# ultravideo/kvazaar

Measured on AMD Instinct MI355X. Metric: CTUs/s (all-intra ultrafast hot path), higher is better.
Workload: dtype u8/i16 (f64 RD costs); 1 GPU; 1920x1080 yuv420p 8-bit all-intra ultrafast CTU pass (kvz_hip_intra_frames), QP 22; ctus_per_frame=510, distinct_frames=8, wpp=True, parallelism=frames sharded over 1 GPU(s), no data-path collective

## Files before the change

include/kvz_hip_dev.h:

```cpp
#ifndef KVZ_HIP_DEV_H_
#define KVZ_HIP_DEV_H_

#include "kvz_hip_types.h"

#ifdef __cplusplus
extern "C" {
#endif

void *kvz_hip_dev_alloc(size_t bytes);
void  kvz_hip_dev_free(void *p);
void  kvz_hip_dev_upload(void *dev_dst, const void *host_src, size_t bytes);
void  kvz_hip_dev_download(void *host_dst, const void *dev_src, size_t bytes);
void  kvz_hip_dev_sync(void);
void  kvz_hip_dev_copy(void *dev_dst, const void *dev_src, size_t bytes);
void  kvz_hip_dev_timer_start(void);
float kvz_hip_dev_timer_stop(void);

int  kvz_hip_dev_sad_nxn(int n, const uint8_t *a, const uint8_t *b, int count, uint32_t *out);
int  kvz_hip_dev_satd_nxn(int n, const uint8_t *a, const uint8_t *b, int count, uint32_t *out);

int  kvz_hip_dev_transform(int kind, const int16_t *in, int16_t *tmp, int16_t *out, int count, int use_matrix_cores);

int  kvz_hip_dev_angular_pred(int log2_width, int mode, const uint8_t *ref_above, const uint8_t *ref_left, int count, uint8_t *out);

int  kvz_hip_dev_intra_select(int log2w, int nblk, const uint32_t *raw, const int8_t *preds, const double *mode_bits, int count, int32_t *winner);

int  kvz_hip_dev_cu8_units(int count, int from_coeffs, const int16_t *in, const int32_t *qp, int16_t *levels, int16_t *dequant, int16_t *resid);

int  kvz_hip_dev_satd8_blocks(const uint8_t *a, const uint8_t *b, int count, uint32_t *out);

int  kvz_hip_dev_rough_rows(int log2w, const uint8_t *top, const uint8_t *left, int count, uint8_t *out);

void kvz_hip_dev_deblock_frames(uint8_t *frames, int width, int height, int n_frames, const uint8_t *cu_depth, int qp, int beta_offset_div2,
                                int tc_offset_div2);

typedef struct kvz_hip_cu_dbk {
  uint8_t type;
  uint8_t depth, tr_depth, part_size;
  uint8_t cbf_y;
  uint8_t mv_dir;
  int8_t  mv_ref[2];
  int16_t ref_id[2];
  int16_t mv[2][2];
} kvz_hip_cu_dbk;
void kvz_hip_dev_deblock_frames_inter(uint8_t *frames, int width, int height, int n_frames, const kvz_hip_cu_dbk *info, int qp, int beta_offset_div2,
                                      int tc_offset_div2, int slice_is_b);

int  kvz_hip_dev_loop_filters_inter(const uint8_t *src, uint8_t *rec, int width, int height, int n_pictures, const kvz_hip_cu_dbk *info, int qp, int slice_is_b, int deblock,
                                    int beta_offset_div2, int tc_offset_div2, int sao, int no_wpp, kvz_hip_sao_params *luma, kvz_hip_sao_params *chroma, uint8_t *merge);

int  kvz_hip_dev_sad_surface(const uint8_t *cur, const uint8_t *ref, int width, int height, int bw, int range, const int16_t *blk_xy, int count,
                             uint32_t *out);

typedef struct kvz_hip_fme_pu {
// ... 123 lines not shown
```

kvazaar_amd/csrc/kvz_ctu.hpp:

```cpp
#pragma once
#include <type_traits>
#include "../../include/kvz_hip_types.h"
#include "kvz_ops.hpp"
#include "kvz_rdoq.hpp"
#include "kvz_recon.hpp"
#include "kvz_residual.hpp"
#include "kvz_select.hpp"

namespace kvz {

#define KVZ_CTU_THREADS 128
#ifdef KVZ_HOSTSIM
#define KVZ_FOR_THREADS(tid) for (int tid = 0; tid < KVZ_CTU_THREADS; ++tid)
#ifdef KVZ_HOSTSIM_COUNT_SYNCS
static unsigned long long g_kvz_syncs;
#define KVZ_SYNC() (++g_kvz_syncs)
#else
#define KVZ_SYNC()
#endif
#define KVZ_LDS_ADD(p, v) (*(p) += (v))
#else
#define KVZ_FOR_THREADS(tid) for (int tid = (threadIdx.x + lane_rot) & (KVZ_CTU_THREADS - 1), once_ = 1; once_; once_ = 0)
#define KVZ_SYNC() __syncthreads()
#define KVZ_LDS_ADD(p, v) atomicAdd((p), (v))
// ... 233 lines not shown
  u8 dcval[3];
  int8_t mode_disp[35];
  int16_t mode_inv[35];
  QuantScalars qs[4][2];
  double mode_bits_cost[3];
  CtxSetT<CABAC> cab, pre[3], post2;
  float entropy_fbits[128];
  u8 ctx_lps[64];
};

using CtuShared = CtuSharedT<true>;
static_assert(__builtin_offsetof(CtuSharedT<true>, fref) == __builtin_offsetof(CtuSharedT<true>, ref) + 408 && __builtin_offsetof(CtuSharedT<false>, fref) == __builtin_offsetof(CtuSharedT<false>, ref) + 408,
              "Tables::mref_tab addresses the filtered references 408 bytes behind the unfiltered ones");
static_assert(KVZ_MREF_STRIDE == kMrefStride && KVZ_MREF_ORG == kMrefOrg && sizeof(((CtuSharedT<true> *)0)->ref[0][0]) == kMrefRefRow && kMrefFiltered == 408,
              "Tables::mref_tab (kvz_tables.hpp) is built for this layout of the reference arrays");
#define KVZ_FROM_REF(T, member) (__builtin_offsetof(T, member) - __builtin_offsetof(T, ref))
static_assert(KVZ_FROM_REF(CtuSharedT<true>, mref) == kMrefExtended && KVZ_FROM_REF(CtuSharedT<false>, mref) == kMrefExtended && KVZ_FROM_REF(CtuSharedT<true>, org_t) == kSatdSrcT &&
              KVZ_FROM_REF(CtuSharedT<false>, org_t) == kSatdSrcT && KVZ_FROM_REF(CtuSharedT<true>, edge_x) == kSatdEdge && KVZ_FROM_REF(CtuSharedT<false>, edge_x) == kSatdEdge,
              "Tables::satd_rows (kvz_tables.hpp) addresses the extended references, the transposed source block and the edge bytes from CtuShared::ref");
static_assert(sizeof(((CtuSharedT<true> *)0)->edge_x) >= 1 + 2 * 16 && __builtin_offsetof(CtuSharedT<true>, edge_x) + sizeof(((CtuSharedT<true> *)0)->edge_x) <= __builtin_offsetof(CtuSharedT<true>, lv2_coeff) &&
              __builtin_offsetof(CtuSharedT<true>, org) == 0 && __builtin_offsetof(CtuSharedT<true>, ref) % 8 == 0 && __builtin_offsetof(CtuSharedT<true>, org_t) % 8 == 0,
              "the edge bytes of a 16x16 CU fit, behind satd_raw and inside the union; source rows (offsets that are multiples of 8 from org / org_t) are 8-byte aligned");
static_assert(__builtin_offsetof(CtuSharedT<true>, lv2_coeff) - __builtin_offsetof(CtuSharedT<true>, tb_big) == 3072 + 1536, "the union is as large as its 32x32 regime: edge_x added nothing");
#undef KVZ_FROM_REF
static_assert(KVZ_CTU_THREADS == 128, "two wavefronts per CTU: thread 64 is 'the other wavefront' (recon_cu8, eval_pu, wide_task, rdoq_unit, prices_coeffs, kHookThread), a 16x16 CU's "
                                      "128 (mode, block) pairs are one round of rough_search, plane_sums routes DPP rows per wavefront, and mref_pre[4] covers Tables::mref_tab's 510 entries");

KVZ_HD int plane_off(int c) { return c ? 3072 + (c << 10) : 0; }

struct RdoqLds {
  i32 ptab[2 * 148];
  u8 diag8[64];
  u8 mode4[4][64][4];
  u8 nb_mode4_left[16];
  u8 c4[96];
  alignas(8) i16 lv4_coeff[96];
  u8 pu_mode[4], pu_cbf[4];
  int pu_cbf_c[2];
  int a3x, a3y, n_pu;
  double split_cost3;
  CtxSetT<true> pre3, post3;
};
template <bool CABAC, bool S32 = false, bool RDOQ = false, bool SH = false, bool LISTS = false> struct CtuProgramT {
  static_assert(!(SH && RDOQ), "kvz_rdoq's own sign hiding is not built");
  static_assert(!(LISTS && (RDOQ || SH)), "scaling lists with kvz_rdoq or sign data hiding are not built");
  using CtxSet = CtxSetT<CABAC>;
// ... 1321 lines not shown
    if (lv == 3) return levels_lds(lv, c);
    return lv == 2 ? s->lv2_coeff + (c == 0 ? 0 : (c == 1 ? 256 : 320))
         : lv == 1 ? s->lv1_coeff + (c == 0 ? 0 : (c == 1 ? 1024 : 1280)) : coeff_level(lv) + plane_off(c) + ctu_zorder(xl >> sh, yl >> sh);
  }

  KVZ_DEV static int wide_trips(int lw) { return lw == 4 ? 1 : 2; }
  KVZ_DEV static RowPlan wide_rows(int lw, int trip) { return lw == 4 ? ROWS_W16 : (trip == 0 ? ROWS_W32_Y : ROWS_W32_C); }
  KVZ_DEV static int wide_task(int lw, int trip, int tid, int *seg)
  {
    *seg = 0;
    if (lw == 4) {
      if (tid < 32) { *seg = tid; return 0; }
      if (tid >= 64 || (tid & 15) >= 8) return -1;
      *seg = tid & 7;
      return tid < 48 ? 1 : 2;
    }
    if (trip == 0) { *seg = tid; return 0; }
    if (tid >= 64) return -1;
    *seg = tid & 31;
    return 1 + (tid >> 5);
  }
  KVZ_DEV void predict_row8(int l2, int mode, int c, int px0, int py, u8 out[8]) const
  {
    const int w = 1 << l2;
    const bool edges = c == 0 && w < 32;
    const u8 *top = s->ref[c][0], *left = s->ref[c][1];
    if (c == 0 && luma_reads_filtered(l2, mode)) { top = s->fref[0]; left = s->fref[1]; }
    if (mode == 0) {
      const int l = left[py + 1], tr = top[w + 1], bl = left[w + 1];
      const int hb = (w - 1) * l + tr + (py + 1) * bl + w, dl = tr - l, wy = w - 1 - py;
      for (int k = 0; k < 8; k++) out[k] = (u8)(((px0 + k) * dl + top[px0 + k + 1] * wy + hb) >> (l2 + 1));
    } else if (mode == 1) {
      const int dc = s->dcval[c];
      for (int k = 0; k < 8; k++) out[k] = (u8)dc;
      if (edges) {
        if (py == 0) for (int k = 0; k < 8; k++) out[k] = (u8)((top[px0 + k + 1] + 3 * dc + 2) >> 2);
        if (px0 == 0) out[0] = (u8)(py == 0 ? (left[1] + 2 * dc + top[1] + 2) >> 2 : (left[py + 1] + 3 * dc + 2) >> 2);
      }
    } else {
      const int disp = s->mode_disp[mode], inv = s->mode_inv[mode];
      const bool vertical = mode >= 18;
      const u8 *main_ref = vertical ? top : left, *side_ref = vertical ? left : top;
      if (vertical) {
        const int delta = (py + 1) * disp, di = delta >> 5, df = delta & 31;
        int r[9];
        if (disp >= 0) for (int j = 0; j < 9; j++) r[j] = main_ref[px0 + di + j + 1];
        else for (int j = 0; j < 9; j++) r[j] = angular_ref(main_ref, side_ref, px0 + di + j, inv);
        for (int k = 0; k < 8; k++) out[k] = (u8)(((32 - df) * r[k] + df * r[k + 1] + 16) >> 5);
        if (edges && mode == 26 && px0 == 0) out[0] = (u8)iclip(0, 255, (int)out[0] + ((left[py + 1] - left[0]) >> 1));
      } else {
        for (int k = 0; k < 8; k++) {
          const int delta = (px0 + k + 1) * disp, di = delta >> 5, df = delta & 31;
          const int r1 = disp >= 0 ? (int)main_ref[py + di + 1] : angular_ref(main_ref, side_ref, py + di, inv);
          const int r2 = disp >= 0 ? (int)main_ref[py + di + 2] : angular_ref(main_ref, side_ref, py + di + 1, inv);
          int v = ((32 - df) * r1 + df * r2 + 16) >> 5;
          if (edges && mode == 10 && py == 0) v = iclip(0, 255, v + ((top[px0 + k + 1] - top[0]) >> 1));
          out[k] = (u8)v;
        }
      }
    }
  }

  KVZ_DEV void predict_chroma_pair(int l2, int mode, int x, int y, u8 *pu, u8 *pv) const
  {
    const u8 *top_u = s->ref[1][0], *left_u = s->ref[1][1], *top_v = s->ref[2][0], *left_v = s->ref[2][1];
    if (mode == 0) { *pu = planar_pixel(l2, x, y, top_u, left_u); *pv = planar_pixel(l2, x, y, top_v, left_v); return; }
    if (mode == 1) { *pu = s->dcval[1]; *pv = s->dcval[2]; return; }
    const bool vertical = mode >= 18;
    const int px = vertical ? x : y, py = vertical ? y : x;
    const int delta_pos = (py + 1) * s->mode_disp[mode], di = delta_pos >> 5, df = delta_pos & 31, inv = s->mode_inv[mode];
    const int i1 = px + di, i2 = i1 + 1;
    const bool main1 = i1 >= -1, main2 = i2 >= -1;
    const int o1 = main1 ? i1 + 1 : (128 + (-1 - i1) * inv) >> 8, o2 = main2 ? i2 + 1 : (128 + (-1 - i2) * inv) >> 8;
    auto plane = [&](const u8 *top, const u8 *left) {
      const u8 *main_ref = vertical ? top : left, *side_ref = vertical ? left : top;
      const int r1 = (main1 ? main_ref : side_ref)[o1], r2 = (main2 ? main_ref : side_ref)[o2];
      return (u8)(((32 - df) * r1 + df * r2 + 16) >> 5);
    };
    *pu = plane(top_u, left_u);
    *pv = plane(top_v, left_v);
  }

  KVZ_DEV void recon_cu16(int lv, const TuSet &t, int depth, int mode)
  {
    const int xl = t.x - cx, yl = t.y - cy, xc = xl >> 1, yc = yl >> 1;
    const CandView cv = cand_view(lv);
    const int umode = uni(mode);
    const bool to_stage = cabac_on() && lv == 0;
    KVZ_LANE_VAR(WideBytes<16>, mat_f);
    KVZ_LANE_VAR(WideBytes<16>, mat_i);
    KVZ_LANE_VAR(u32, pred_org);
    KVZ_LANE_VAR(u32, coded);
#ifdef KVZ_HOSTSIM
#define KVZ_CU16_CODED(tid, c) ((void)KVZ_LANE(coded, tid), s->acc[6 + (c)] != 0)
#else
#define KVZ_CU16_CODED(tid, c) (((KVZ_LANE(coded, tid) >> ((c) == 2 ? 1 : 0)) & 1u) != 0)
#endif
    KVZ_FOR_THREADS(tid) {
      if (tid < 3) s->acc[3 * tid] = 0;
      if (tid >= 64 && tid < 70) s->acc[1 + (tid - 64) + ((tid - 64) >> 1)] = 0;
      if (tid < 32) {
        const int seg = mover_lane(tid), py = seg >> 1, px0 = (seg << 3) & 15;
        u8 p[8], o[8];
        i16 res[8];
        predict_row8(4, umode, 0, px0, py, p);
        __builtin_memcpy(o, KVZ_ALIGNED(org_at(0, xl + px0, yl + py), 8), 8);
        for (int k = 0; k < 8; k++) res[k] = (i16)((int)o[k] - (int)p[k]);
        __builtin_memcpy(KVZ_ALIGNED(&cv.at(0, xl + px0, yl + py), 8), p, 8);
        __builtin_memcpy(KVZ_ALIGNED(tbuf(t, 0, 0) + (seg << 3), 16), res, 16);
      } else if (tid >= 64) {
        const int e = tid - 64, px = e & 7, py = e >> 3;
        cu8_matrix_rows<3>(tb, e, KVZ_LANE(mat_f, tid), KVZ_LANE(mat_i, tid));
        u8 pu, pv;
        predict_chroma_pair(3, umode, px, py, &pu, &pv);
        cv.at(1, xc + px, yc + py) = pu;
        cv.at(2, xc + px, yc + py) = pv;
        const u8 ou = *org_at(1, xc + px, yc + py), ov = *org_at(2, xc + px, yc + py);
        KVZ_LANE(pred_org, tid) = (u32)pu | ((u32)ou << 8) | ((u32)pv << 16) | ((u32)ov << 24);
        tbuf(t, 0, 1)[e] = (i16)((int)ou - (int)pu);
        tbuf(t, 0, 2)[e] = (i16)((int)ov - (int)pv);
      }
    }
    KVZ_WAVE_SYNC();
    KVZ_PROF(KVZ_P_RPRED);
    KVZ_FOR_THREADS(tid) {
      if (tid < 64) transform_big(4, tbuf(t, 0, 0), false, tid, 0);
      else {
        const int e = tid - 64;
        tbuf(t, 1, 1)[e] = cu8_fwd_first<3>(tbuf(t, 0, 1), e, KVZ_LANE(mat_f, tid));
        tbuf(t, 1, 2)[e] = cu8_fwd_first<3>(tbuf(t, 0, 2), e, KVZ_LANE(mat_f, tid));
      }
    }
    KVZ_WAVE_SYNC();
    KVZ_PROF(KVZ_P_FDCT);
    KVZ_FOR_THREADS(tid) {
      const u32 cw_lo = (u32)uni((int)(u32)m->coeff_weights), cw_hi = (u32)uni((int)(u32)(m->coeff_weights >> 32));
      if (tid < 64) {
        u32 packed = 0;
        if (tid < 32) {
          const int seg = mover_lane(tid);
          const QuantScalars q = s->qs[2][0];
          i16 cf[8], lvl[8], dq[8];
          __builtin_memcpy(cf, KVZ_ALIGNED(tbuf(t, 0, 0) + (seg << 3), 16), 16);
          u32 wsum = 0, nz = 0;
          for (int k = 0; k < 8; k++) {
            ListFactor f{ 0, 0 };
            if constexpr (LISTS) f = factor_at(0, 4, (seg << 3) + k);
            const int level = LISTS ? quant_level(cf[k], q, f.fwd) : quant_level(cf[k], q);
            lvl[k] = (i16)level;
            const LevelCost lc = level_cost(level, cw_lo, cw_hi);
            wsum += lc.weight;
            nz += lc.nonzero;
            dq[k] = LISTS ? dequant_level(level, q, f.inv) : dequant_level(level, q);
          }
          packed = wsum | (nz << 24);
          __builtin_memcpy(KVZ_ALIGNED(coeff_dst(lv, 0, xl, yl) + (seg << 3), 16), lvl, 16);
          if (to_stage) __builtin_memcpy(KVZ_ALIGNED(levels_lds(lv, 0) + (seg << 3), 16), lvl, 16);
          __builtin_memcpy(KVZ_ALIGNED(tbuf(t, 1, 0) + (seg << 3), 16), dq, 16);
        }
        KVZ_LANE(coded, tid) = plane_sums(ROWS_CU16, tid, tid < 32 ? 0 : -1, packed, true, 3) != 0;
      } else {
        const int e = tid - 64;
        const QuantScalars q = s->qs[1][1];
        auto plane = [&](int c) {
          const int cf = cu8_fwd_second<3>(tbuf(t, 1, c), e, KVZ_LANE(mat_f, tid));
          ListFactor f{ 0, 0 };
          if constexpr (LISTS) f = factor_at(c, 3, e);
          const int level = LISTS ? quant_level(cf, q, f.fwd) : quant_level(cf, q);
          coeff_dst(lv, c, xl, yl)[e] = (i16)level;
          if (to_stage) levels_lds(lv, c)[e] = (i16)level;
          tbuf(t, 0, c)[cu8_transposed<3>(e)] = LISTS ? dequant_level(level, q, f.inv) : dequant_level(level, q);
          return level_cost(level, cw_lo, cw_hi).word();
        };
        const u32 wu = plane(1), wv = plane(2);
        const u32 nu = plane_sums(ROWS_CU16, tid, 1, wu, true, 3), nv = plane_sums(ROWS_CU16, tid, 2, wv, true, 3);
        KVZ_LANE(coded, tid) = (u32)(nu != 0) | ((u32)(nv != 0) << 1);
      }
    }
    KVZ_WAVE_SYNC();
    KVZ_PROF(KVZ_P_QUANT);
    KVZ_FOR_THREADS(tid) {
      if (tid < 64) { if (uni((int)KVZ_CU16_CODED(tid, 0))) transform_big(4, tbuf(t, 1, 0), true, tid, 0); }
      else {
        const int e = tid - 64;
        if (KVZ_CU16_CODED(tid, 1)) tbuf(t, 1, 1)[cu8_transposed<3>(e)] = cu8_inv_first<3>(tbuf(t, 0, 1), e, KVZ_LANE(mat_i, tid));
        if (KVZ_CU16_CODED(tid, 2)) tbuf(t, 1, 2)[cu8_transposed<3>(e)] = cu8_inv_first<3>(tbuf(t, 0, 2), e, KVZ_LANE(mat_i, tid));
      }
    }
    KVZ_WAVE_SYNC();
    KVZ_PROF(KVZ_P_IDCT);
    KVZ_FOR_THREADS(tid) {
      if (tid < 64) {
        u32 ssd = 0;
        if (tid < 32) {
          const int seg = mover_lane(tid), py = seg >> 1, px0 = (seg << 3) & 15;
          u8 *rp = &cv.at(0, xl + px0, yl + py);
          u8 v[8], o[8];
          __builtin_memcpy(v, KVZ_ALIGNED(rp, 8), 8);
          __builtin_memcpy(o, KVZ_ALIGNED(org_at(0, xl + px0, yl + py), 8), 8);
          if (KVZ_CU16_CODED(tid, 0)) {
            i16 res[8];
            __builtin_memcpy(res, KVZ_ALIGNED(tbuf(t, 1, 0) + (seg << 3), 16), 16);
            for (int k = 0; k < 8; k++) v[k] = (u8)recon_sample(v[k], res[k]);
            __builtin_memcpy(KVZ_ALIGNED(rp, 8), v, 8);
          }
          for (int k = 0; k < 8; k++) ssd += sq_err(o[k], v[k]);
        }
        plane_sums(ROWS_CU16, tid, tid < 32 ? 0 : -1, ssd, false, 0);
      } else {
        const int e = tid - 64, px = e & 7, py = e >> 3;
        auto plane = [&](int c) {
          const u32 po = KVZ_LANE(pred_org, tid) >> (c == 2 ? 16 : 0);
          int v = (int)(po & 0xffu);
          if (KVZ_CU16_CODED(tid, c)) {
            v = recon_sample(v, cu8_inv_second<3>(tbuf(t, 1, c), e, KVZ_LANE(mat_i, tid)));
            cv.at(c, xc + px, yc + py) = (u8)v;
          }
          return sq_err((int)((po >> 8) & 0xffu), v);
        };
        const u32 su = plane(1), sv = plane(2);
        plane_sums(ROWS_CU16, tid, 1, su, false, 0);
        plane_sums(ROWS_CU16, tid, 2, sv, false, 0);
      }
    }
#undef KVZ_CU16_CODED
    KVZ_SYNC();
    KVZ_FOR_THREADS(tid) {
      if (tid == 0) finish_planes(lv, xl, yl, depth, 0, 3, false);
    }
    if (cabac_on()) KVZ_SYNC();
    KVZ_PROF(KVZ_P_RECON);
// ... 23 lines not shown
          i16 res[8];
          predict_row8(l2, umode, c, px0, py, p);
          __builtin_memcpy(o, KVZ_ALIGNED(org_at(c, (xl >> sh) + px0, (yl >> sh) + py), 8), 8);
          for (int k = 0; k < 8; k++) res[k] = (i16)((int)o[k] - (int)p[k]);
          __builtin_memcpy(KVZ_ALIGNED(&cv.at(c, (xl >> sh) + px0, (yl >> sh) + py), 8), p, 8);
          __builtin_memcpy(KVZ_ALIGNED(tbuf(t, 0, c) + (seg << 3), 16), res, 16);
        }
      }
    } else
    KVZ_FOR_THREADS(tid) {
      if (tid < 16) s->acc[tid] = 0;
      for (int c = 0; c < 3; c++) {
        const int l2 = tu_log2(t, c), w = 1 << l2, sh = c ? 1 : 0;
        for (int e = tid; e < w * w; e += KVZ_CTU_THREADS) {
          const int px = e & (w - 1), py = e >> l2;
          const u8 p = predict_pixel(l2, mode, c, px, py);
          cv.at(c, (xl >> sh) + px, (yl >> sh) + py) = p;
          tbuf(t, 0, c)[e] = (i16)((int)*org_at(c, (xl >> sh) + px, (yl >> sh) + py) - (int)p);
        }
      }
    }
    KVZ_SYNC();
    KVZ_PROF(KVZ_P_RPRED);
    for (int pass = 0; pass < 2; pass++) {
      KVZ_FOR_THREADS(tid) {
        for (int c = 0; c < 3; c++) {
          const int l2 = tu_log2(t, c), n = 1 << l2;
          const i16 *src = tbuf(t, pass, c);
          i16 *dst = tbuf(t, pass ^ 1, c);
          if (l2 >= 4) {
            if (pass == 0 && !(big_pairs(t) && c == 2)) transform_big(l2, tbuf(t, 0, c), false, tid, c, big_pairs(t) && c == 1);
            continue;
          }
          for (int e = tid; e < n * n; e += KVZ_CTU_THREADS) {
            const int k = e >> l2, j = e & (n - 1);
            dst[e] = fwd_point(n, [&](int i) { return dct_at(l2, k, i); }, src, j << l2, pass == 0 ? l2 - 1 : l2 + 6);
          }
        }
      }
      KVZ_SYNC();
    }
    KVZ_PROF(KVZ_P_FDCT);
    if (RDOQ && m->rdoq) {
      KVZ_FOR_THREADS(tid) { rdoq_unit(tid, lv, t, true, depth, mode); }
      KVZ_SYNC();
      KVZ_PROF(KVZ_P_RDOQ);
    }
    if (SH && !RDOQ && wide && hide_on()) {
      auto held = [&](int c) { return lv == 0 ? levels_lds(lv, c) : coeff_dst(lv, c, xl, yl); };
      KVZ_FOR_THREADS(tid) {
        for (int trip = 0; trip < wide_trips(t.lw); trip++) {
          int seg;
          const int c = wide_task(t.lw, trip, mover_lane(tid), &seg);
          if (c < 0) continue;
          const QuantScalars q = s->qs[tu_log2(t, c) - 2][c ? 1 : 0];
          i16 cf[8], lvl[8];
          __builtin_memcpy(cf, KVZ_ALIGNED(tbuf(t, 0, c) + (seg << 3), 16), 16);
          for (int k = 0; k < 8; k++) lvl[k] = (i16)quant_level(cf[k], q);
          __builtin_memcpy(KVZ_ALIGNED(held(c) + (seg << 3), 16), lvl, 16);
        }
      }
      KVZ_SYNC();
      KVZ_FOR_THREADS(tid) { hide_signs(tid, t.lw, tu_log2(t, 1), intra_scan_order(mode, depth), tbuf(t, 0, 0), held(0), tbuf(t, 0, 1), held(1), tbuf(t, 0, 2), held(2)); }
// ... 79 lines not shown
        block_add(&s->acc[3 + c], wsum);
        block_add(&s->acc[6 + c], nz);
      }
    }
    KVZ_SYNC();
    KVZ_PROF(KVZ_P_QUANT);
    for (int pass = 0; pass < 2; pass++) {
      KVZ_FOR_THREADS(tid) {
        for (int c = 0; c < 3; c++) {
          const int l2 = tu_log2(t, c), n = 1 << l2;
          if (!s->acc[6 + c]) continue;
          const i16 *src = tbuf(t, pass ^ 1, c);
          i16 *dst = tbuf(t, pass, c);
          if (l2 >= 4) {
            if (pass == 0 && !(big_pairs(t) && c == 2 && s->acc[7])) transform_big(l2, tbuf(t, 1, c), true, tid, c, big_pairs(t) && c == 1 && s->acc[8]);
            continue;
          }
          for (int e = tid; e < n * n; e += KVZ_CTU_THREADS) {
            const int j = e >> l2, i = e & (n - 1);
            dst[e] = inv_point(n, [&](int k) { return dct_at(l2, k, i); }, src, j, n, pass == 0 ? 7 : 12);
          }
        }
      }
      KVZ_SYNC();
    }
    KVZ_PROF(KVZ_P_IDCT);
    KVZ_FOR_THREADS(tid) {
      if (wide) {
        for (int trip = 0; trip < wide_trips(t.lw); trip++) {
          int seg;
          const int c = wide_task(t.lw, trip, mover_lane(tid), &seg);
          u32 ssd = 0;
          if (c >= 0) {
            const int l2 = tu_log2(t, c), sh = c ? 1 : 0, py = seg >> (l2 - 3), px0 = (seg << 3) & ((1 << l2) - 1);
            u8 *rp = &cv.at(c, (xl >> sh) + px0, (yl >> sh) + py);
            u8 v[8], o[8];
            __builtin_memcpy(v, KVZ_ALIGNED(rp, 8), 8);
            __builtin_memcpy(o, KVZ_ALIGNED(org_at(c, (xl >> sh) + px0, (yl >> sh) + py), 8), 8);
            if (s->acc[6 + c] != 0) {
              i16 res[8];
              __builtin_memcpy(res, KVZ_ALIGNED(tbuf(t, 1, c) + (seg << 3), 16), 16);
              for (int k = 0; k < 8; k++) v[k] = (u8)recon_sample(v[k], res[k]);
              __builtin_memcpy(KVZ_ALIGNED(rp, 8), v, 8);
            }
            for (int k = 0; k < 8; k++) ssd += sq_err(o[k], v[k]);
          }
          plane_sums(wide_rows(t.lw, trip), tid, c, ssd, false, 0);
// ... 1106 lines not shown
```

kvazaar_amd/csrc/kvz_dev.hpp:

```cpp
#pragma once
#include <hip/hip_runtime.h>

#include <functional>
#include <mutex>
#include <chrono>
#include <vector>

#include "../../include/kvz_hip_dev.h"
#include "kvz_mfma.hpp"
#include "kvz_ops.hpp"
#include "kvz_sao.hpp"
#include "kvz_entropy.hpp"
#include "kvz_select.hpp"
#include "kvz_recon.hpp"
#include "kvz_tables.hpp"

namespace kvz {

__device__ __forceinline__ u32 load_u32_any(const u8 *p) { u32 v; __builtin_memcpy(&v, p, 4); return v; }
template <int G> __device__ __forceinline__ u32 group_sum(u32 v)
{
  for (int off = G / 2; off > 0; off >>= 1) v += __shfl_down(v, off, G);
  return v;
}
// ... 309 lines not shown
      const u8 xv = satd_edge_byte(ref0, L2, tid & (2 * W - 1));
      ref0[kSatdEdge + (tid == 2 * W ? 0 : 1 + tid)] = tid == 2 * W ? (u8)0 : xv;
    }
  }
  __syncthreads();
  if (!live || (L2 == 3 && tid >= 64)) return;
#pragma unroll
  for (int j = 0; j < (L2 == 4 ? 2 : 1); j++) {
    const int g = L2 == 4 ? 2 * (tid >> 6) + j : 0, pr = 32 * g + (lane & 31), mode = 2 + (pr >> LB), b = pr & (NBLK - 1);
    const dev_int4 *row = reinterpret_cast<const dev_int4 *>(tb->satd_rows[L2 == 4 ? 1 + g : 0][lane]);
    const dev_int4 e[2] = { row[0], row[1] };
    dev_int4 p[2];
    satd_rows_predict(ref0, e, p);
    u8 *o = out + ((cu * 32 + (mode - 2)) * NBLK + b) * 64;
#pragma unroll
    for (int i = 0; i < 4; i++)
#pragma unroll
      for (int x = 0; x < 8; x++) {
        const int r = 4 * (lane >> 5) + i;
        const u8 v = (u8)(((u32)p[i >> 1][2 * (i & 1) + (x >> 2)] >> (8 * (x & 3))) ^ 0x80);
        o[mode >= 18 ? 8 * r + x : 8 * x + r] = v;
      }
  }
}

template <int L2> __global__ void __launch_bounds__(256) dev_angular_kernel(const u8 *above, const u8 *left, const int count, const int mode, u8 *out)
{
  constexpr int W = 1 << L2, NG = kAngularGroupsPerLane, GPB = W * W / 4, BLOCKS = 256 * NG / GPB, RS = 2 * W + 1, ES = (2 * W + 1 + 8 + 3) & ~3;
  constexpr int RAW = (BLOCKS * RS + 3 + 3) / 4 + 2;
  __shared__ u32 s_raw[2][RAW];
  __shared__ alignas(8) u8 s_ext[BLOCKS][ES];
  __shared__ u32 s_tile[BLOCKS * W * W / 4];
  const int disp_tab[9] = { 0, 2, 5, 9, 13, 17, 21, 26, 32 };
  const int inv_tab[9] = { 0, 4096, 1638, 910, 630, 482, 390, 315, 256 };
  const bool vertical = mode >= 18;
  const int mode_disp = vertical ? mode - 26 : 10 - mode, ad = iabs(mode_disp);
  const int disp = mode_disp < 0 ? -disp_tab[ad] : disp_tab[ad], inv = inv_tab[ad];
  const long blk0 = (long)blockIdx.x * BLOCKS;
  const int nblk = (int)(count - blk0 < BLOCKS ? count - blk0 : BLOCKS);
  const long g0 = blk0 * RS;
  const int mis = (int)(g0 & 3), ndw = (mis + nblk * RS + 3) >> 2;
  const u8 *main_g = vertical ? above : left, *side_g = vertical ? left : above;
  const int tid = threadIdx.x;
  for (int i = tid; i < ndw; i += 256) {
    s_raw[0][i] = reinterpret_cast<const u32 *>(main_g + g0 - mis)[i];
    if (disp < 0) s_raw[1][i] = reinterpret_cast<const u32 *>(side_g + g0 - mis)[i];
// ... 857 lines not shown
}

int kvz_hip_dev_intra_select(int log2w, int nblk, const uint32_t *raw, const int8_t *preds, const double *mode_bits, int count, int32_t *winner)
{
  if (!((log2w == 3 && nblk == 1) || (log2w == 4 && nblk == 4))) { fprintf(stderr, "kvz_hip_dev_intra_select: unsupported log2w=%d nblk=%d\n", log2w, nblk); return -1; }
  if (count <= 0) return 0;
  KVZ_DEV_LAUNCH(kvz::dev_intra_select_kernel, ((long)count + 3) / 4 * 256, raw, preds, mode_bits, count, log2w, nblk, winner);
  return 0;
}

int kvz_hip_dev_cu8_units(int count, int from_coeffs, const int16_t *in, const int32_t *qp, int16_t *levels, int16_t *dequant, int16_t *resid)
{
  if (count < 0 || (from_coeffs != 0 && from_coeffs != 1)) { fprintf(stderr, "kvz_hip_dev_cu8_units: count=%d from_coeffs=%d\n", count, from_coeffs); return -1; }
  if (count == 0) return 0;
  KVZ_DEV_LAUNCH(kvz::dev_cu8_units_kernel, ((long)count + 1) / 2 * 256, in, qp, count, from_coeffs, kvz::device_tables(), levels, dequant, resid);
  return 0;
}

int kvz_hip_dev_rough_rows(int log2w, const uint8_t *top, const uint8_t *left, int count, uint8_t *out)
{
  if (count < 0 || (log2w != 3 && log2w != 4)) { fprintf(stderr, "kvz_hip_dev_rough_rows: log2w=%d count=%d\n", log2w, count); return -1; }
  if (log2w == 3) KVZ_DEV_LAUNCH(kvz::dev_rough_rows_kernel<3>, ((long)count + 1) / 2 * 256, kvz::device_tables(), top, left, count, out);
  else KVZ_DEV_LAUNCH(kvz::dev_rough_rows_kernel<4>, ((long)count + 1) / 2 * 256, kvz::device_tables(), top, left, count, out);
  return 0;
}

int kvz_hip_dev_satd8_blocks(const uint8_t *a, const uint8_t *b, int count, uint32_t *out)
{
  if (count < 0) { fprintf(stderr, "kvz_hip_dev_satd8_blocks: count=%d\n", count); return -1; }
  KVZ_DEV_LAUNCH(kvz::dev_satd8_blocks_kernel, ((long)count + 31) / 32 * 64, kvz::device_tables(), a, b, count, out);
  return 0;
}

void kvz_hip_dev_deblock_frames(uint8_t *frames, int width, int height, int n_frames, const uint8_t *cu_depth, int qp, int beta_offset_div2,
                                int tc_offset_div2)
{
  kvz::deblock_frames_on(be().stream, frames, width, height, n_frames, cu_depth, qp, beta_offset_div2, tc_offset_div2);
}

void kvz_hip_dev_deblock_frames_inter(uint8_t *frames, int width, int height, int n_frames, const kvz_hip_cu_dbk *info, int qp, int beta_offset_div2, int tc_offset_div2,
                                      int slice_is_b)
{
  kvz::deblock_frames_on(be().stream, frames, width, height, n_frames, nullptr, qp, beta_offset_div2, tc_offset_div2, 3, info, slice_is_b);
}

namespace kvz {
// ... 1027 lines not shown
```

kvazaar_amd/csrc/kvz_ops.hpp:

```cpp
#pragma once
#include <stdint.h>

#ifdef KVZ_HOSTSIM
#define KVZ_DEV inline
#define KVZ_ATOMIC_ADD(p, v) (*(p) += (v))
#else
#include <hip/hip_runtime.h>
#define KVZ_DEV __device__ __forceinline__
#define KVZ_ATOMIC_ADD(p, v) atomicAdd((p), (v))
#endif

namespace kvz {

typedef uint8_t u8;
typedef int16_t i16;
typedef uint16_t u16;
typedef uint32_t u32;
typedef int32_t i32;

#ifdef KVZ_HOSTSIM
#define KVZ_HD inline
#else
#define KVZ_HD __host__ __device__ __forceinline__
#endif
// ... 459 lines not shown
        const int scanpos = cg * cg_size + in_cg;
        const u32 blkpos = scan[scanpos];
        const int qv = quant_coeff[blkpos];
        int ld = imin(iabs((int)coef[blkpos]) * qv, 0x7fffffff - (1 << (q_bits - 1)));
        const u32 mx = (u32)((ld + (1 << (q_bits - 1))) >> q_bits);
        if (mx > 0) {
          res[0] = scanpos; res[1] = cg; res[2] = cg; res[3] = (scanpos > 0 && type == 0) ? 2 : 0; res[4] = (i32)blkpos;
          return;
        }
        dest[blkpos] = 0;
      }
    }
    res[2] = cg;
  }
};


KVZ_DEV int angular_ref(const u8 *main_ref, const u8 *side_ref, int i, int inv)
{
  const u8 *p = i >= -1 ? main_ref + (i + 1) : side_ref + ((128 + (-1 - i) * inv) >> 8);
  return *p;
}

KVZ_DEV u8 angular_pixel(int mode, int x, int y, const u8 *above, const u8 *left)
{
  const int disp_tab[9] = { 0, 2, 5, 9, 13, 17, 21, 26, 32 };
  const int inv_tab[9] = { 0, 4096, 1638, 910, 630, 482, 390, 315, 256 };
  const bool vertical = mode >= 18;
  const int mode_disp = vertical ? mode - 26 : 10 - mode;
  const int ad = iabs(mode_disp);
  const int sample_disp = mode_disp < 0 ? -disp_tab[ad] : disp_tab[ad];
  const u8 *main_ref = vertical ? above : left, *side_ref = vertical ? left : above;
  const int px = vertical ? x : y, py = vertical ? y : x;
  if (sample_disp == 0) return main_ref[px + 1];
  const int delta_pos = (py + 1) * sample_disp;
  const int di = delta_pos >> 5, df = delta_pos & 31;
  const int inv = inv_tab[ad];
  const int r1 = angular_ref(main_ref, side_ref, px + di, inv);
  if (!df) return (u8)r1;
  const int r2 = angular_ref(main_ref, side_ref, px + di + 1, inv);
  return (u8)(((32 - df) * r1 + df * r2 + 16) >> 5);
}

KVZ_DEV u8 planar_pixel(int log2w, int x, int y, const u8 *top, const u8 *left)
{
  const int w = 1 << log2w;
  const int hor = (w - 1 - x) * left[y + 1] + (x + 1) * top[w + 1];
  const int ver = (w - 1 - y) * top[x + 1] + (y + 1) * left[w + 1];
  return (u8)((ver + hor + w) >> (log2w + 1));
}

KVZ_DEV int dc_value(int log2w, const u8 *top, const u8 *left)
{
  const int w = 1 << log2w;
  int sum = 0;
  for (int i = 0; i < w; i++) sum += top[i + 1] + left[i + 1];
  return (u8)((sum + w) >> (log2w + 1));
}

KVZ_DEV u8 filtered_dc_pixel(int dc, int x, int y, const u8 *top, const u8 *left)
{
  if (x == 0 && y == 0) return (u8)((left[1] + 2 * dc + top[1] + 2) / 4);
  if (y == 0) return (u8)((top[x + 1] + 3 * dc + 2) / 4);
  if (x == 0) return (u8)((left[y + 1] + 3 * dc + 2) / 4);
  return (u8)dc;
}

struct IntraPredOp {
  int kind, log2w; const int8_t *modes ; const u8 *above; const u8 *left; long ref_bstride; u8 *dst;
  KVZ_DEV void operator()(int item) const
  {
    const int w = 1 << log2w, blk = item >> (2 * log2w), e = item & (w * w - 1), y = e >> log2w, x = e & (w - 1);
    const u8 *t = above + blk * ref_bstride, *l = left + blk * ref_bstride;
    u8 v;
    if (kind == 0) v = angular_pixel(modes[blk], x, y, t, l);
    else if (kind >= 3) v = angular_pixel(kind - 3, x, y, t, l);
    else if (kind == 1) v = planar_pixel(log2w, x, y, t, l);
    else v = filtered_dc_pixel(dc_value(log2w, t, l), x, y, t, l);
    dst[item] = v;
  }
};

KVZ_DEV int hor8(const int8_t *f, const u8 *src, int stride, int r, int c)
{
  const u8 *p = src + (long)r * stride + c - 3;
  int t = 0;
  for (int i = 0; i < 8; i++) t += f[i] * (int)p[i];
  return t;
}
KVZ_DEV int hv8(const int8_t *hf, const int8_t *vf, const u8 *src, int stride, int r, int c)
// ... 135 lines not shown
```

kvazaar_amd/csrc/kvz_recon.hpp:

```cpp
#pragma once
#include "kvz_ops.hpp"
#include "kvz_syntax.hpp"

namespace kvz {

KVZ_HD bool luma_reads_filtered(int log2w, int mode)
{
  if (mode == 1 || log2w == 2) return false;
  return mode == 0 || imin(iabs(mode - 26), iabs(mode - 10)) > (log2w == 3 ? 7 : (log2w == 4 ? 1 : 0));
}

template <class Mat> KVZ_DEV i16 fwd_point(int n, Mat m, const i16 *in, int at, int shift)
{
  int a = 0;
  for (int i = 0; i < n; i++) a += m(i) * (int)in[at + i];
  return (i16)((a + (1 << (shift - 1))) >> shift);
}
template <class Mat> KVZ_DEV i16 inv_point(int n, Mat m, const i16 *in, int at, int stride, int shift)
{
  int a = 0;
  for (int k = 0; k < n; k++) a += m(k) * (int)in[k * stride + at];
  return (i16)iclip(-32768, 32767, (a + (1 << (shift - 1))) >> shift);
}

template <int N, class Row, class MatRow> KVZ_DEV int row_dot(const Row &x, const MatRow &m)
{
  int a = 0;
  for (int i = 0; i < N / 2; i++) a = dot2_i16(x.w[i], m.w[i], a);
  return a;
}
template <int N, class Row, class MatRow> KVZ_DEV i16 fwd_row_point(const Row &x, const MatRow &m, int shift) { return (i16)((row_dot<N>(x, m) + (1 << (shift - 1))) >> shift); }
template <int N, class Row, class MatRow> KVZ_DEV i16 inv_row_point(const Row &x, const MatRow &m, int shift)
// ... 131 lines not shown
```

kvazaar_amd/dev.py:

```python
import ctypes as C

import numpy as np

TRANSFORM_KINDS = {"dct4": 0, "dct8": 1, "dct16": 2, "dct32": 3, "dst4": 4, "idct4": 5, "idct8": 6, "idct16": 7, "idct32": 8, "idst4": 9}
TRANSFORM_SIZE = {0: 4, 1: 8, 2: 16, 3: 32, 4: 4, 5: 4, 6: 8, 7: 16, 8: 32, 9: 4}


class Dev:
    def __init__(self, cdll):
        self.lib = l = cdll
        vp, sz, ci = C.c_void_p, C.c_size_t, C.c_int
        l.kvz_hip_dev_alloc.restype = vp; l.kvz_hip_dev_alloc.argtypes = [sz]
        l.kvz_hip_dev_free.restype = None; l.kvz_hip_dev_free.argtypes = [vp]
        l.kvz_hip_dev_upload.restype = None; l.kvz_hip_dev_upload.argtypes = [vp, vp, sz]
        l.kvz_hip_dev_download.restype = None; l.kvz_hip_dev_download.argtypes = [vp, vp, sz]
        l.kvz_hip_dev_sync.restype = None; l.kvz_hip_dev_sync.argtypes = []
        l.kvz_hip_dev_timer_start.restype = None; l.kvz_hip_dev_timer_start.argtypes = []
        l.kvz_hip_dev_timer_stop.restype = C.c_float; l.kvz_hip_dev_timer_stop.argtypes = []
        for f in (l.kvz_hip_dev_sad_nxn, l.kvz_hip_dev_satd_nxn):
            f.restype = None; f.argtypes = [ci, vp, vp, ci, vp]
        l.kvz_hip_dev_transform.restype = None; l.kvz_hip_dev_transform.argtypes = [ci, vp, vp, vp, ci, ci]
        l.kvz_hip_dev_angular_pred.restype = None; l.kvz_hip_dev_angular_pred.argtypes = [ci, ci, vp, vp, ci, vp]
        l.kvz_hip_dev_intra_select.restype = ci; l.kvz_hip_dev_intra_select.argtypes = [ci, ci, vp, vp, vp, ci, vp]
        l.kvz_hip_dev_cu8_units.restype = ci; l.kvz_hip_dev_cu8_units.argtypes = [ci, ci, vp, vp, vp, vp, vp]
        l.kvz_hip_dev_satd8_blocks.restype = ci; l.kvz_hip_dev_satd8_blocks.argtypes = [vp, vp, ci, vp]
        if hasattr(l, "kvz_hip_dev_rough_rows"):
            l.kvz_hip_dev_rough_rows.restype = ci; l.kvz_hip_dev_rough_rows.argtypes = [ci, vp, vp, ci, vp]

    def put(self, a):
        a = np.ascontiguousarray(a)
        p = self.lib.kvz_hip_dev_alloc(a.nbytes)
        self.lib.kvz_hip_dev_upload(p, a.ctypes.data, a.nbytes)
        return p

    def copy_in(self, p, a):
        a = np.ascontiguousarray(a)
        self.lib.kvz_hip_dev_upload(p, a.ctypes.data, a.nbytes)

    def empty(self, nbytes):
        return self.lib.kvz_hip_dev_alloc(nbytes)

    def get(self, p, shape, dtype):
        out = np.empty(shape, dtype)
        self.lib.kvz_hip_dev_download(out.ctypes.data, p, out.nbytes)
        return out

    def free(self, *ps):
        for p in ps:
            self.lib.kvz_hip_dev_free(p)
```

Baseline: 3.579 million CTUs/s.

## Spread 16x16 CU luma prediction, quant and recon over a full wavefront

The 16x16 CU luma path (predict/residual, quant/dequant, recon/SSD) now uses all 64 lanes of the first wavefront with 4-sample segments, where it used 32 lanes with 8 samples each. Prediction reads the precomputed extended angular references (mref) instead of projecting samples per pixel, and static asserts guarantee that reconstruction leaves those buffers intact. A barrier in the chroma-pair transform passes is skipped for large CUs. A standalone cu16 predict kernel and its binding are added for testing. The change trades more lanes and narrower memory accesses for shorter per-lane serial work, and it relies on mref being valid at recon time.

```diff
diff --git a/include/kvz_hip_dev.h b/include/kvz_hip_dev.h
--- a/include/kvz_hip_dev.h
+++ b/include/kvz_hip_dev.h
@@ -30,6 +30,8 @@
 int  kvz_hip_dev_satd8_blocks(const uint8_t *a, const uint8_t *b, int count, uint32_t *out);
 
 int  kvz_hip_dev_rough_rows(int log2w, const uint8_t *top, const uint8_t *left, int count, uint8_t *out);
+
+int  kvz_hip_dev_cu16_predict(const uint8_t *top, const uint8_t *left, const uint8_t *modes, int count, uint8_t *out);
 
 void kvz_hip_dev_deblock_frames(uint8_t *frames, int width, int height, int n_frames, const uint8_t *cu_depth, int qp, int beta_offset_div2,
                                 int tc_offset_div2);
diff --git a/kvazaar_amd/csrc/kvz_ctu.hpp b/kvazaar_amd/csrc/kvz_ctu.hpp
--- a/kvazaar_amd/csrc/kvz_ctu.hpp
+++ b/kvazaar_amd/csrc/kvz_ctu.hpp
@@ -279,6 +279,13 @@
               __builtin_offsetof(CtuSharedT<true>, org) == 0 && __builtin_offsetof(CtuSharedT<true>, ref) % 8 == 0 && __builtin_offsetof(CtuSharedT<true>, org_t) % 8 == 0,
               "the edge bytes of a 16x16 CU fit, behind satd_raw and inside the union; source rows (offsets that are multiples of 8 from org / org_t) are 8-byte aligned");
 static_assert(__builtin_offsetof(CtuSharedT<true>, lv2_coeff) - __builtin_offsetof(CtuSharedT<true>, tb_big) == 3072 + 1536, "the union is as large as its 32x32 regime: edge_x added nothing");
+static_assert(__builtin_offsetof(CtuSharedT<true>, mref) >= __builtin_offsetof(CtuSharedT<true>, c2) + sizeof(((CtuSharedT<true> *)0)->c2) &&
+              __builtin_offsetof(CtuSharedT<true>, c2) >= __builtin_offsetof(CtuSharedT<true>, tb_small) + sizeof(((CtuSharedT<true> *)0)->tb_small) &&
+              __builtin_offsetof(CtuSharedT<true>, mref) + sizeof(((CtuSharedT<true> *)0)->mref) <= __builtin_offsetof(CtuSharedT<true>, edge_x) &&
+              __builtin_offsetof(CtuSharedT<true>, edge_x) + sizeof(((CtuSharedT<true> *)0)->edge_x) <= __builtin_offsetof(CtuSharedT<true>, lv2_coeff) &&
+              __builtin_offsetof(CtuSharedT<false>, mref) >= __builtin_offsetof(CtuSharedT<false>, c2) + sizeof(((CtuSharedT<false> *)0)->c2) &&
+              __builtin_offsetof(CtuSharedT<false>, edge_x) + sizeof(((CtuSharedT<false> *)0)->edge_x) <= __builtin_offsetof(CtuSharedT<false>, lv2_coeff),
+              "CtuShared::mref and edge_x lie behind the two transform buffers and the depth-2 candidate and in front of lv2_coeff: a 16x16 CU's reconstruction leaves them alone");
 #undef KVZ_FROM_REF
 static_assert(KVZ_CTU_THREADS == 128, "two wavefronts per CTU: thread 64 is 'the other wavefront' (recon_cu8, eval_pu, wide_task, rdoq_unit, prices_coeffs, kHookThread), a 16x16 CU's "
                                       "128 (mode, block) pairs are one round of rough_search, plane_sums routes DPP rows per wavefront, and mref_pre[4] covers Tables::mref_tab's 510 entries");
@@ -1646,43 +1653,15 @@
   }
   KVZ_DEV void predict_row8(int l2, int mode, int c, int px0, int py, u8 out[8]) const
   {
-    const int w = 1 << l2;
-    const bool edges = c == 0 && w < 32;
-    const u8 *top = s->ref[c][0], *left = s->ref[c][1];
-    if (c == 0 && luma_reads_filtered(l2, mode)) { top = s->fref[0]; left = s->fref[1]; }
-    if (mode == 0) {
-      const int l = left[py + 1], tr = top[w + 1], bl = left[w + 1];
-      const int hb = (w - 1) * l + tr + (py + 1) * bl + w, dl = tr - l, wy = w - 1 - py;
-      for (int k = 0; k < 8; k++) out[k] = (u8)(((px0 + k) * dl + top[px0 + k + 1] * wy + hb) >> (l2 + 1));
-    } else if (mode == 1) {
-      const int dc = s->dcval[c];
-      for (int k = 0; k < 8; k++) out[k] = (u8)dc;
-      if (edges) {
-        if (py == 0) for (int k = 0; k < 8; k++) out[k] = (u8)((top[px0 + k + 1] + 3 * dc + 2) >> 2);
-        if (px0 == 0) out[0] = (u8)(py == 0 ? (left[1] + 2 * dc + top[1] + 2) >> 2 : (left[py + 1] + 3 * dc + 2) >> 2);
-      }
-    } else {
-      const int disp = s->mode_disp[mode], inv = s->mode_inv[mode];
-      const bool vertical = mode >= 18;
-      const u8 *main_ref = vertical ? top : left, *side_ref = vertical ? left : top;
-      if (vertical) {
-        const int delta = (py + 1) * disp, di = delta >> 5, df = delta & 31;
-        int r[9];
-        if (disp >= 0) for (int j = 0; j < 9; j++) r[j] = main_ref[px0 + di + j + 1];
-        else for (int j = 0; j < 9; j++) r[j] = angular_ref(main_ref, side_ref, px0 + di + j, inv);
-        for (int k = 0; k < 8; k++) out[k] = (u8)(((32 - df) * r[k] + df * r[k + 1] + 16) >> 5);
-        if (edges && mode == 26 && px0 == 0) out[0] = (u8)iclip(0, 255, (int)out[0] + ((left[py + 1] - left[0]) >> 1));
-      } else {
-        for (int k = 0; k < 8; k++) {
-          const int delta = (px0 + k + 1) * disp, di = delta >> 5, df = delta & 31;
-          const int r1 = disp >= 0 ? (int)main_ref[py + di + 1] : angular_ref(main_ref, side_ref, py + di, inv);
-          const int r2 = disp >= 0 ? (int)main_ref[py + di + 2] : angular_ref(main_ref, side_ref, py + di + 1, inv);
-          int v = ((32 - df) * r1 + df * r2 + 16) >> 5;
-          if (edges && mode == 10 && py == 0) v = iclip(0, 255, v + ((top[px0 + k + 1] - top[0]) >> 1));
-          out[k] = (u8)v;
-        }
-      }
-    }
+    RowRefs rr;
+    rr.top = s->ref[c][0]; rr.left = s->ref[c][1];
+    if (c == 0 && luma_reads_filtered(l2, mode)) { rr.top = s->fref[0]; rr.left = s->fref[1]; }
+    rr.edges = c == 0 && l2 < 5;
+    rr.dc = mode == 1 ? (int)s->dcval[c] : 0;
+    rr.disp = mode >= 2 ? (int)s->mode_disp[mode] : 0;
+    rr.inv = mode >= 2 ? (int)s->mode_inv[mode] : 0;
+    rr.ext = nullptr;
+    predict_row_segment<8, false>(l2, mode, rr, px0, py, out);
   }
 
   KVZ_DEV void predict_chroma_pair(int l2, int mode, int x, int y, u8 *pu, u8 *pv) const
@@ -1723,16 +1702,16 @@
     KVZ_FOR_THREADS(tid) {
       if (tid < 3) s->acc[3 * tid] = 0;
       if (tid >= 64 && tid < 70) s->acc[1 + (tid - 64) + ((tid - 64) >> 1)] = 0;
-      if (tid < 32) {
-        const int seg = mover_lane(tid), py = seg >> 1, px0 = (seg << 3) & 15;
-        u8 p[8], o[8];
-        i16 res[8];
-        predict_row8(4, umode, 0, px0, py, p);
-        __builtin_memcpy(o, KVZ_ALIGNED(org_at(0, xl + px0, yl + py), 8), 8);
-        for (int k = 0; k < 8; k++) res[k] = (i16)((int)o[k] - (int)p[k]);
-        __builtin_memcpy(KVZ_ALIGNED(&cv.at(0, xl + px0, yl + py), 8), p, 8);
-        __builtin_memcpy(KVZ_ALIGNED(tbuf(t, 0, 0) + (seg << 3), 16), res, 16);
-      } else if (tid >= 64) {
+      if (tid < 64) {
+        const int seg = mover_lane(tid), py = cu16_luma_segment(seg).py, px0 = cu16_luma_segment(seg).px0;
+        u8 p[4], o[4];
+        i16 res[4];
+        cu16_predict_lane(&s->ref[0][0][0], umode, umode == 1 ? (int)s->dcval[0] : 0, umode >= 2 ? (int)s->mode_disp[umode] : 0, umode >= 2 ? (int)s->mode_inv[umode] : 0, seg, p);
+        __builtin_memcpy(o, KVZ_ALIGNED(org_at(0, xl + px0, yl + py), 4), 4);
+        for (int k = 0; k < 4; k++) res[k] = (i16)((int)o[k] - (int)p[k]);
+        __builtin_memcpy(KVZ_ALIGNED(&cv.at(0, xl + px0, yl + py), 4), p, 4);
+        __builtin_memcpy(KVZ_ALIGNED(tbuf(t, 0, 0) + (seg << 2), 8), res, 8);
+      } else {
         const int e = tid - 64, px = e & 7, py = e >> 3;
         cu8_matrix_rows<3>(tb, e, KVZ_LANE(mat_f, tid), KVZ_LANE(mat_i, tid));
         u8 pu, pv;
@@ -1760,29 +1739,26 @@
     KVZ_FOR_THREADS(tid) {
       const u32 cw_lo = (u32)uni((int)(u32)m->coeff_weights), cw_hi = (u32)uni((int)(u32)(m->coeff_weights >> 32));
       if (tid < 64) {
-        u32 packed = 0;
-        if (tid < 32) {
-          const int seg = mover_lane(tid);
-          const QuantScalars q = s->qs[2][0];
-          i16 cf[8], lvl[8], dq[8];
-          __builtin_memcpy(cf, KVZ_ALIGNED(tbuf(t, 0, 0) + (seg << 3), 16), 16);
-          u32 wsum = 0, nz = 0;
-          for (int k = 0; k < 8; k++) {
-            ListFactor f{ 0, 0 };
-            if constexpr (LISTS) f = factor_at(0, 4, (seg << 3) + k);
-            const int level = LISTS ? quant_level(cf[k], q, f.fwd) : quant_level(cf[k], q);
-            lvl[k] = (i16)level;
-            const LevelCost lc = level_cost(level, cw_lo, cw_hi);
-            wsum += lc.weight;
-            nz += lc.nonzero;
-            dq[k] = LISTS ? dequant_level(level, q, f.inv) : dequant_level(level, q);
-          }
-          packed = wsum | (nz << 24);
-          __builtin_memcpy(KVZ_ALIGNED(coeff_dst(lv, 0, xl, yl) + (seg << 3), 16), lvl, 16);
-          if (to_stage) __builtin_memcpy(KVZ_ALIGNED(levels_lds(lv, 0) + (seg << 3), 16), lvl, 16);
-          __builtin_memcpy(KVZ_ALIGNED(tbuf(t, 1, 0) + (seg << 3), 16), dq, 16);
-        }
-        KVZ_LANE(coded, tid) = plane_sums(ROWS_CU16, tid, tid < 32 ? 0 : -1, packed, true, 3) != 0;
+        const int seg = mover_lane(tid);
+        const QuantScalars q = s->qs[2][0];
+        i16 cf[4], lvl[4], dq[4];
+        __builtin_memcpy(cf, KVZ_ALIGNED(tbuf(t, 0, 0) + (seg << 2), 8), 8);
+        u32 wsum = 0, nz = 0;
+        for (int k = 0; k < 4; k++) {
+          ListFactor f{ 0, 0 };
+          if constexpr (LISTS) f = factor_at(0, 4, (seg << 2) + k);
+          const int level = LISTS ? quant_level(cf[k], q, f.fwd) : quant_level(cf[k], q);
+          lvl[k] = (i16)level;
+          const LevelCost lc = level_cost(level, cw_lo, cw_hi);
+          wsum += lc.weight;
+          nz += lc.nonzero;
+          dq[k] = LISTS ? dequant_level(level, q, f.inv) : dequant_level(level, q);
+        }
+        const u32 packed = wsum | (nz << 24);
+        __builtin_memcpy(KVZ_ALIGNED(coeff_dst(lv, 0, xl, yl) + (seg << 2), 8), lvl, 8);
+        if (to_stage) __builtin_memcpy(KVZ_ALIGNED(levels_lds(lv, 0) + (seg << 2), 8), lvl, 8);
+        __builtin_memcpy(KVZ_ALIGNED(tbuf(t, 1, 0) + (seg << 2), 8), dq, 8);
+        KVZ_LANE(coded, tid) = plane_sums(ROWS_CU16, tid, 0, packed, true, 3) != 0;
       } else {
         const int e = tid - 64;
         const QuantScalars q = s->qs[1][1];
@@ -1816,21 +1792,19 @@
     KVZ_FOR_THREADS(tid) {
       if (tid < 64) {
         u32 ssd = 0;
-        if (tid < 32) {
-          const int seg = mover_lane(tid), py = seg >> 1, px0 = (seg << 3) & 15;
-          u8 *rp = &cv.at(0, xl + px0, yl + py);
-          u8 v[8], o[8];
-          __builtin_memcpy(v, KVZ_ALIGNED(rp, 8), 8);
-          __builtin_memcpy(o, KVZ_ALIGNED(org_at(0, xl + px0, yl + py), 8), 8);
-          if (KVZ_CU16_CODED(tid, 0)) {
-            i16 res[8];
-            __builtin_memcpy(res, KVZ_ALIGNED(tbuf(t, 1, 0) + (seg << 3), 16), 16);
-            for (int k = 0; k < 8; k++) v[k] = (u8)recon_sample(v[k], res[k]);
-            __builtin_memcpy(KVZ_ALIGNED(rp, 8), v, 8);
-          }
-          for (int k = 0; k < 8; k++) ssd += sq_err(o[k], v[k]);
-        }
-        plane_sums(ROWS_CU16, tid, tid < 32 ? 0 : -1, ssd, false, 0);
+        const int seg = mover_lane(tid), py = cu16_luma_segment(seg).py, px0 = cu16_luma_segment(seg).px0;
+        u8 *rp = &cv.at(0, xl + px0, yl + py);
+        u8 v[4], o[4];
+        __builtin_memcpy(v, KVZ_ALIGNED(rp, 4), 4);
+        __builtin_memcpy(o, KVZ_ALIGNED(org_at(0, xl + px0, yl + py), 4), 4);
+        if (KVZ_CU16_CODED(tid, 0)) {
+          i16 res[4];
+          __builtin_memcpy(res, KVZ_ALIGNED(tbuf(t, 1, 0) + (seg << 2), 8), 8);
+          for (int k = 0; k < 4; k++) v[k] = (u8)recon_sample(v[k], res[k]);
+          __builtin_memcpy(KVZ_ALIGNED(rp, 4), v, 4);
+        }
+        for (int k = 0; k < 4; k++) ssd += sq_err(o[k], v[k]);
+        plane_sums(ROWS_CU16, tid, 0, ssd, false, 0);
       } else {
         const int e = tid - 64, px = e & 7, py = e >> 3;
         auto plane = [&](int c) {
@@ -1900,6 +1874,7 @@
     }
     KVZ_SYNC();
     KVZ_PROF(KVZ_P_RPRED);
+    const int passes = t.lc >= 4 ? 1 : 2;
     for (int pass = 0; pass < 2; pass++) {
       KVZ_FOR_THREADS(tid) {
         for (int c = 0; c < 3; c++) {
@@ -1916,7 +1891,7 @@
           }
         }
       }
-      KVZ_SYNC();
+      if (pass < passes) KVZ_SYNC();
     }
     KVZ_PROF(KVZ_P_FDCT);
     if (RDOQ && m->rdoq) {
@@ -2042,7 +2017,7 @@
           }
         }
       }
-      KVZ_SYNC();
+      if (pass < passes) KVZ_SYNC();
     }
     KVZ_PROF(KVZ_P_IDCT);
     KVZ_FOR_THREADS(tid) {
diff --git a/kvazaar_amd/csrc/kvz_dev.hpp b/kvazaar_amd/csrc/kvz_dev.hpp
--- a/kvazaar_amd/csrc/kvz_dev.hpp
+++ b/kvazaar_amd/csrc/kvz_dev.hpp
@@ -355,6 +355,35 @@
         o[mode >= 18 ? 8 * r + x : 8 * x + r] = v;
       }
   }
+}
+
+__global__ void __launch_bounds__(256) dev_cu16_predict_kernel(const Tables *tb, const u8 *top, const u8 *left, const u8 *modes, const int count, u8 *out)
+{
+  constexpr int W = 16, N = 2 * W + 1, NM = (15 * (2 * W + 2) + 127) / 128;
+  static_assert(2 * N <= 128 && NM * 128 <= 512, "a lane per reference sample; Tables::mref_tab rows");
+  __shared__ alignas(16) u8 lds[2][(kMrefExtended + 15 * kMrefStride + 15) & ~15u];
+  const int half = threadIdx.x >> 7, tid = threadIdx.x & 127;
+  const long cu = 2l * blockIdx.x + half;
+  const bool live = cu < count;
+  u8 *ref0 = lds[half];
+  const int side = tid >= N, k = side ? tid - N : tid;
+  if (live && tid < 2 * N) ref0[kMrefRefRow * side + k] = (side ? left : top)[cu * N + k];
+  __syncthreads();
+  if (live && tid < 2 * N) ref0[kMrefFiltered + kMrefRefRow * side + k] = luma_filtered_ref(ref0, N, tid);
+  __syncthreads();
+  if (live) {
+    u32 e[NM];
+    for (int j = 0; j < NM; j++) e[j] = tb->mref_tab[1][tid + j * 128];
+    mref_copy<NM>(ref0, e);
+  }
+  __syncthreads();
+  if (!live || tid >= 64) return;
+  const int mode = imin(modes[cu], 34);
+  int disp, inv;
+  angular_params(mode, &disp, &inv);
+  alignas(4) u8 p[4];
+  cu16_predict_lane(ref0, mode, dc_value(4, ref0, ref0 + kMrefRefRow), disp, inv, tid, p);
+  __builtin_memcpy(__builtin_assume_aligned(out + cu * (W * W) + 4 * tid, 4), p, 4);
 }
 
 template <int L2> __global__ void __launch_bounds__(256) dev_angular_kernel(const u8 *above, const u8 *left, const int count, const int mode, u8 *out)
@@ -1258,6 +1287,13 @@
   if (count < 0 || (log2w != 3 && log2w != 4)) { fprintf(stderr, "kvz_hip_dev_rough_rows: log2w=%d count=%d\n", log2w, count); return -1; }
   if (log2w == 3) KVZ_DEV_LAUNCH(kvz::dev_rough_rows_kernel<3>, ((long)count + 1) / 2 * 256, kvz::device_tables(), top, left, count, out);
   else KVZ_DEV_LAUNCH(kvz::dev_rough_rows_kernel<4>, ((long)count + 1) / 2 * 256, kvz::device_tables(), top, left, count, out);
+  return 0;
+}
+
+int kvz_hip_dev_cu16_predict(const uint8_t *top, const uint8_t *left, const uint8_t *modes, int count, uint8_t *out)
+{
+  if (count < 0) { fprintf(stderr, "kvz_hip_dev_cu16_predict: count=%d\n", count); return -1; }
+  KVZ_DEV_LAUNCH(kvz::dev_cu16_predict_kernel, ((long)count + 1) / 2 * 256, kvz::device_tables(), top, left, modes, count, out);
   return 0;
 }
 
diff --git a/kvazaar_amd/csrc/kvz_ops.hpp b/kvazaar_amd/csrc/kvz_ops.hpp
--- a/kvazaar_amd/csrc/kvz_ops.hpp
+++ b/kvazaar_amd/csrc/kvz_ops.hpp
@@ -505,6 +505,15 @@
   return *p;
 }
 
+KVZ_DEV void angular_params(int mode, int *disp, int *inv)
+{
+  const int disp_tab[9] = { 0, 2, 5, 9, 13, 17, 21, 26, 32 };
+  const int inv_tab[9] = { 0, 4096, 1638, 910, 630, 482, 390, 315, 256 };
+  const int md = mode >= 18 ? mode - 26 : 10 - mode, ad = iabs(md);
+  *disp = mode < 2 ? 0 : (md < 0 ? -disp_tab[ad] : disp_tab[ad]);
+  *inv = mode < 2 ? 0 : inv_tab[ad];
+}
+
 KVZ_DEV u8 angular_pixel(int mode, int x, int y, const u8 *above, const u8 *left)
 {
   const int disp_tab[9] = { 0, 2, 5, 9, 13, 17, 21, 26, 32 };
@@ -549,6 +558,48 @@
   return (u8)dc;
 }
 
+struct RowRefs { const u8 *top, *left, *ext; int dc, disp, inv; bool edges; };
+template <int N, bool EXT> KVZ_DEV void predict_row_segment(int l2, int mode, const RowRefs &rr, int px0, int py, u8 *out)
+{
+  const int w = 1 << l2;
+  const u8 *top = rr.top, *left = rr.left;
+  if (mode == 0) {
+    const int l = left[py + 1], tr = top[w + 1], bl = left[w + 1];
+    const int hb = (w - 1) * l + tr + (py + 1) * bl + w, dl = tr - l, wy = w - 1 - py;
+    for (int k = 0; k < N; k++) out[k] = (u8)(((px0 + k) * dl + top[px0 + k + 1] * wy + hb) >> (l2 + 1));
+  } else if (mode == 1) {
+    const int dc = rr.dc;
+    for (int k = 0; k < N; k++) out[k] = (u8)dc;
+    if (rr.edges) {
+      if (py == 0) for (int k = 0; k < N; k++) out[k] = (u8)((top[px0 + k + 1] + 3 * dc + 2) >> 2);
+      if (px0 == 0) out[0] = (u8)(py == 0 ? (left[1] + 2 * dc + top[1] + 2) >> 2 : (left[py + 1] + 3 * dc + 2) >> 2);
+    }
+  } else {
+    const int disp = rr.disp, inv = rr.inv;
+    const bool vertical = mode >= 18;
+    const u8 *main_ref = vertical ? top : left, *side_ref = vertical ? left : top;
+    const u8 *ext = rr.ext;
+    if (vertical) {
+      const int delta = (py + 1) * disp, di = delta >> 5, df = delta & 31;
+      int r[N + 1];
+      if (disp >= 0) for (int j = 0; j <= N; j++) r[j] = main_ref[px0 + di + j + 1];
+      else if (EXT) for (int j = 0; j <= N; j++) r[j] = ext[px0 + di + j + 1];
+      else for (int j = 0; j <= N; j++) r[j] = angular_ref(main_ref, side_ref, px0 + di + j, inv);
+      for (int k = 0; k < N; k++) out[k] = (u8)(((32 - df) * r[k] + df * r[k + 1] + 16) >> 5);
+      if (rr.edges && mode == 26 && px0 == 0) out[0] = (u8)iclip(0, 255, (int)out[0] + ((left[py + 1] - left[0]) >> 1));
+    } else {
+      for (int k = 0; k < N; k++) {
+        const int delta = (px0 + k + 1) * disp, di = delta >> 5, df = delta & 31;
+        const int r1 = disp >= 0 ? (int)main_ref[py + di + 1] : (EXT ? (int)ext[py + di + 1] : angular_ref(main_ref, side_ref, py + di, inv));
+        const int r2 = disp >= 0 ? (int)main_ref[py + di + 2] : (EXT ? (int)ext[py + di + 2] : angular_ref(main_ref, side_ref, py + di + 1, inv));
+        int v = ((32 - df) * r1 + df * r2 + 16) >> 5;
+        if (rr.edges && mode == 10 && py == 0) v = iclip(0, 255, v + ((top[px0 + k + 1] - top[0]) >> 1));
+        out[k] = (u8)v;
+      }
+    }
+  }
+}
+
 struct IntraPredOp {
   int kind, log2w; const int8_t *modes ; const u8 *above; const u8 *left; long ref_bstride; u8 *dst;
   KVZ_DEV void operator()(int item) const
diff --git a/kvazaar_amd/csrc/kvz_recon.hpp b/kvazaar_amd/csrc/kvz_recon.hpp
--- a/kvazaar_amd/csrc/kvz_recon.hpp
+++ b/kvazaar_amd/csrc/kvz_recon.hpp
@@ -8,6 +8,24 @@
 {
   if (mode == 1 || log2w == 2) return false;
   return mode == 0 || imin(iabs(mode - 26), iabs(mode - 10)) > (log2w == 3 ? 7 : (log2w == 4 ? 1 : 0));
+}
+
+KVZ_DEV RowRefs searched_luma_refs(const u8 *ref0, int log2w, int mode, int dc, int disp, int inv)
+{
+  RowRefs rr;
+  const unsigned set = luma_reads_filtered(log2w, mode) ? kMrefFiltered : 0u;
+  rr.top = ref0 + set; rr.left = ref0 + set + kMrefRefRow;
+  rr.ext = mode >= 11 && mode <= 25 ? ref0 + kMrefExtended + kMrefStride * (unsigned)(mode - 11) + kMrefOrg : nullptr;
+  rr.dc = dc; rr.disp = disp; rr.inv = inv;
+  rr.edges = true;
+  return rr;
+}
+struct RowSegment { int py, px0; };
+KVZ_HD RowSegment cu16_luma_segment(int lane) { RowSegment g; g.py = lane >> 2; g.px0 = (lane & 3) << 2; return g; }
+KVZ_DEV void cu16_predict_lane(const u8 *ref0, int mode, int dc, int disp, int inv, int lane, u8 out[4])
+{
+  const RowSegment g = cu16_luma_segment(lane);
+  predict_row_segment<4, true>(4, mode, searched_luma_refs(ref0, 4, mode, dc, disp, inv), g.px0, g.py, out);
 }
 
 template <class Mat> KVZ_DEV i16 fwd_point(int n, Mat m, const i16 *in, int at, int shift)
diff --git a/kvazaar_amd/dev.py b/kvazaar_amd/dev.py
--- a/kvazaar_amd/dev.py
+++ b/kvazaar_amd/dev.py
@@ -26,6 +26,8 @@
         l.kvz_hip_dev_satd8_blocks.restype = ci; l.kvz_hip_dev_satd8_blocks.argtypes = [vp, vp, ci, vp]
         if hasattr(l, "kvz_hip_dev_rough_rows"):
             l.kvz_hip_dev_rough_rows.restype = ci; l.kvz_hip_dev_rough_rows.argtypes = [ci, vp, vp, ci, vp]
+        if hasattr(l, "kvz_hip_dev_cu16_predict"):
+            l.kvz_hip_dev_cu16_predict.restype = ci; l.kvz_hip_dev_cu16_predict.argtypes = [vp, vp, vp, ci, vp]
 
     def put(self, a):
         a = np.ascontiguousarray(a)
```

Result: faster. 3.658 million CTUs/s (median of 6 runs) (+2.2%).
